# qwerty35/lsc_dr_planner

Hardware: AMD Instinct MI355X
Metric: qp_solves_per_sec (higher is better)
Workload: dtype f64; 1 GPU; configs[1]: 64 agents x M=5 x ~20 LSC half-spaces/seg, fp64 -- 64 agents/GPU x M=5 segments x 20 LSC neighbours (dim=3, forest swarm after 3 warm-up replans), fp64: dual active-set phase (one workgroup per QP) with the batched PDIP behind it for what it leaves; batch_seed=1000, precision=f64, row_format=f64, collective_backend=none (single process), agents_per_gpu=64, agents_total=64, ranks=1, distinct_devices=1, launch=single process, segments=5, lsc_neighbours=20, dim=3, rows_per_qp=1074, allgather=False, pipeline=False, hip_graph=False

## Files before the change

lsc_dr_planner_amd/csrc/lscqp_api.hip:

```cpp
#include <hip/hip_runtime.h>

#include <cmath>
#include <cstdio>
#include <cstdlib>
#include <cstring>
#include <algorithm>
#include <atomic>
#include <mutex>
#include <string>
#include <vector>

#include "lscqp_kernel.hpp"
#include "lscqp_launch.hpp"
#include "lscqp_staging.hpp"
#include "lscqp_internal.hpp"

#define LSCQP_DECL(M, D, E, S, W, X)                                                                                      \
    extern "C" hipError_t lscqp_launch_##M##_##D##_##E##_##S##_##W##_##X(const lscqp::DevClass*, int64_t, const lscqp_header*, \
                                                                  const lscqp_row*, const uint64_t*, const lscqp_box*,  \
                                                                  const double*, double*, double*, int32_t*, lscqp_info*, \
                                                                  hipStream_t);
LSCQP_INSTANCES(LSCQP_DECL)
#undef LSCQP_DECL

// ... 352 lines not shown
        c.dQ[i] = d->control_input_weight != 0
                      ? (double)(((long double)p_ref - (long double)d->control_input_weight * kQInt[i] * scl) /
                                 (long double)d->control_input_weight)
                      : 0.0;
    }
    for (int k = 0; k < 3; k++) {
        c.world_min[k] = d->world_min[k];
        c.world_max[k] = d->world_max[k];
    }
    c.tol = d->tol > 0 ? d->tol : 1e-10;
    c.max_iter = d->max_iter > 0 ? d->max_iter : 60;
    c.use_sfc = d->use_sfc;
    c.n_obs_max = 0;
    c.rows_f32 = d->row_format == LSCQP_ROWS_F32;
    c.repair = 0;
    c.rsfc = d->planner_mode == LSCQP_PLANNER_RSFC;
    if (d->active_set != LSCQP_ACTIVE_SET_DEFAULT && d->active_set != LSCQP_ACTIVE_SET_OFF && d->active_set != LSCQP_ACTIVE_SET_ONLY)
        return fail(LSCQP_ERR_INVALID_ARGUMENT, "active_set must be LSCQP_ACTIVE_SET_DEFAULT, _OFF or _ONLY");
    if (d->warm_start != LSCQP_WARM_DEFAULT && d->warm_start != LSCQP_WARM_TIGHT)
        return fail(LSCQP_ERR_INVALID_ARGUMENT, "warm_start must be LSCQP_WARM_DEFAULT or LSCQP_WARM_TIGHT");
    c.warm_mu0 = d->warm_start == LSCQP_WARM_TIGHT ? 1e-7 : LSCQP_WARM_MU0;
    c.warm_s0 = d->warm_start == LSCQP_WARM_TIGHT ? 0.003 : LSCQP_WARM_S0;
    c.warm_net = d->warm_start == LSCQP_WARM_TIGHT ? 0.6 : 0.0;
    return LSCQP_OK;
}

extern "C" const lscqp_class_desc* lscqp_class_desc_of_(lscqp_handle h) { return &h->desc; }
extern "C" uint64_t lscqp_handle_generation_(lscqp_handle h) { return h->generation; }

static bool das_upload(DasTables& D, int d) {
    if (D.dev[d]) {
        D.garbage.push_back({D.dev[d], d});
        D.dev[d] = nullptr;
    }
    if (D.host.empty()) return false;
    if (hipSetDevice(d) != hipSuccess) return false;
    double* p = nullptr;
    if (hipMalloc(&p, sizeof(double) * D.host.size()) != hipSuccess) return false;
    if (hipMemcpy(p, D.host.data(), sizeof(double) * D.host.size(), hipMemcpyHostToDevice) != hipSuccess) {
        (void)hipFree(p);
        return false;
    }
    D.dev[d] = p;
    D.dev_n[d] = D.host.size();
    D.dev_gen[d] = D.gen;
    return true;
}
static void das_refresh(lscqp_solver* s) {
    if (!s->das) return;
    std::lock_guard<std::mutex> lk(s->das->mu);
    DasTables& D = *s->das;
    const size_t nd = lscqp_das_build_tables(s->desc.M, s->es, s->desc.dt, s->desc.control_input_weight, s->desc.terminal_weight, nullptr);
    const size_t npair = lscqp_das_build_pairs(s->desc.M, s->desc.dim, s->desc.communication_range > 0, nullptr);
    std::vector<double> fresh(nd + 36 + npair, 0.0);
    if (s->desc.control_input_weight > 0 && s->desc.terminal_weight >= 0 &&
        lscqp_das_build_tables(s->desc.M, s->es, s->desc.dt, s->desc.control_input_weight, s->desc.terminal_weight, fresh.data()) == nd) {
        for (int i = 0; i < 36; i++) fresh[nd + i] = s->dev.dQ[i];
        static_assert(sizeof(double) == 2 * sizeof(int32_t), "two ints per table slot");
        lscqp_das_build_pairs(s->desc.M, s->desc.dim, s->desc.communication_range > 0, reinterpret_cast<int32_t*>(fresh.data() + nd + 36));
    } else {
        fresh.clear();
    }
    if (D.gen != 0 && fresh.size() == D.host.size() && (fresh.empty() || memcmp(fresh.data(), D.host.data(), sizeof(double) * fresh.size()) == 0))
        return;
    D.host.swap(fresh);
    D.gen++;
    int cur = 0;
    const bool have_cur = hipGetDevice(&cur) == hipSuccess;
    for (int d = 0; d < 64; d++)
        if (D.dev[d]) (void)das_upload(D, d);
    if (D.garbage.size() > DasTables::kMaxRetired) {
        for (const DasTables::Retired& g : D.garbage) {
            if (hipSetDevice(g.dev) == hipSuccess) {
                (void)hipDeviceSynchronize();
                (void)hipFree(g.p);
            }
        }
        D.garbage.clear();
    }
    if (have_cur) (void)hipSetDevice(cur);
}
static const double* das_device_table(lscqp_solver* s, hipStream_t stream, int* err = nullptr) {
    if (err) *err = 0;
    if (!s->das) return nullptr;
    int dev = 0;
    if (hipGetDevice(&dev) != hipSuccess || dev < 0 || dev >= 64) return nullptr;
    std::lock_guard<std::mutex> lk(s->das->mu);
    DasTables& D = *s->das;
    if (D.host.empty()) return nullptr;
    if (D.dev[dev] && D.dev_gen[dev] == D.gen) return D.dev[dev];
    hipStreamCaptureStatus cap = hipStreamCaptureStatusNone;
    const hipError_t qe = hipStreamIsCapturing(stream, &cap);
    if (qe != hipSuccess) (void)hipGetLastError();
    const bool capturing = qe != hipSuccess || cap != hipStreamCaptureStatusNone;
    if (capturing) {
        if (err) *err = 2;
        return nullptr;
    }
    if (!das_upload(D, dev)) {
        if (err) *err = 1;
        return nullptr;
    }
    return D.dev[dev];
}

static inline size_t row_bytes(lscqp_handle h) { return h->dev.rows_f32 ? sizeof(lscqp_row_f32) : sizeof(lscqp_row); }

extern "C" {

int lscqp_create(const lscqp_class_desc* desc, lscqp_handle* out) {
    if (!desc || !out) return fail(LSCQP_ERR_INVALID_ARGUMENT, "null argument");
    lscqp_solver* s = new lscqp_solver();
// ... 508 lines not shown
```

lsc_dr_planner_amd/csrc/lscqp_das.hip:

```cpp
#include <hip/hip_runtime.h>
#include <stdint.h>

#include <atomic>
#include <cmath>
#include <mutex>
#include <vector>

#include "lscqp_internal.hpp"
#include "lscqp_das.hpp"


extern "C" size_t lscqp_das_build_pairs(int M, int dim, int comm_on, int32_t* out) {
    const int P = 6 * M, NX = dim * P, NCP = M * (M - 1) / 2;
    const int oV = NX, oA = oV + dim * 5 * M, oC = oA + dim * 4 * M, NPAIR = lscqp_das::num_pairs(M, dim);
    if (!out) return (size_t)NPAIR;
    for (int r = 0; r < NPAIR; r++) {
        int type = 0, e0 = 0, e1 = 0, fam = 0, k = 0, m = 0, last = 0;
        if (r < oV) {
            k = r / P;
            const int cp = r - k * P;
            m = cp / 6, last = cp % 6 == 5;
            type = cp >= 3 ? 1 : 0, e0 = r, fam = 0;
        } else if (r < oA) {
            const int s = r - oV;
            k = s / (5 * M);
            const int rr = s - k * 5 * M, i = rr % 5;
            m = rr / 5;
            type = (m == 0 && i < 2) ? 0 : 2, e0 = k * P + 6 * m + i, fam = 1;
        } else if (r < oC) {
            const int s = r - oA;
            k = s / (4 * M);
            const int rr = s - k * 4 * M, i = rr % 4;
            m = rr / 4;
            type = (m == 0 && i < 1) ? 0 : 3, e0 = k * P + 6 * m + i, fam = 2;
        } else {
            const int s = r - oC;
            k = s / NCP;
            const int ci = s - k * NCP;
            int uu = 1;
            while (uu * (uu + 1) / 2 <= ci) uu++;
            const int up = ci - uu * (uu - 1) / 2;
            type = comm_on ? 4 : 0, e0 = k * P + 6 * (up + 1), e1 = k * P + 6 * uu + 5, fam = 3, m = 0;
        }
        out[2 * r] = (type << 24) | (e0 << 12) | e1;
        out[2 * r + 1] = fam | (k << 2) | (m << 4) | (last << 8) | ((fam == 0 && k == 2 && m == 0) ? 1 << 9 : 0);
    }
    return (size_t)NPAIR;
}

extern "C" size_t lscqp_das_build_tables(int M, int es, double dt, double w_c, double w_t, double* out) {
    const int P = 6 * M, NZA = 3 * (M - 1) + (es ? 1 : 3);
    const size_t stride = lscqp_das::table_stride(M);
    if (!out) return stride * (size_t)M;
    typedef long double ld;
    const ld q2s = 2.0L * (ld)w_c / ((ld)dt * dt * dt * dt * dt);
    static const int kq[6][6] = {{720, -1800, 1200, 0, 0, -120},  {-1800, 4800, -3600, 0, 600, 0}, {1200, -3600, 3600, -1200, 0, 0},
                                 {0, 0, -1200, 3600, -3600, 1200}, {0, 600, 0, -3600, 4800, -1800}, {-120, 0, 0, 1200, -1800, 720}};
    static const int tbm[3][3] = {{0, 0, 1}, {0, -1, 2}, {1, -4, 4}};
    std::vector<ld> Tm((size_t)P * NZA, 0.0L);
    for (int m = 0; m < M; m++) {
        const bool last = es && m == M - 1;
        for (int j = 0; j < 3; j++) Tm[(size_t)(6 * m + 3 + j) * NZA + 3 * m + (last ? 0 : j)] = 1.0L;
        if (m >= 1)
            for (int i = 0; i < 3; i++)
                for (int j = 0; j < 3; j++) Tm[(size_t)(6 * m + i) * NZA + 3 * (m - 1) + j] = (ld)tbm[i][j];
    }
    for (int ts = 1; ts <= M; ts++) {
        std::vector<ld> Hx((size_t)P * P, 0.0L);
        for (int m = 0; m < M; m++)
            for (int i = 0; i < 6; i++)
                for (int j = 0; j < 6; j++) Hx[(size_t)(6 * m + i) * P + 6 * m + j] += q2s * (ld)kq[i][j];
        for (int m = M - ts; m < M; m++) Hx[(size_t)(6 * m + 5) * P + 6 * m + 5] += 2.0L * (ld)w_t;
        std::vector<ld> HT((size_t)P * NZA, 0.0L), K0((size_t)NZA * NZA, 0.0L);
        for (int i = 0; i < P; i++)
            for (int l = 0; l < P; l++) {
                const ld h = Hx[(size_t)i * P + l];
                if (h == 0.0L) continue;
                for (int j = 0; j < NZA; j++) HT[(size_t)i * NZA + j] += h * Tm[(size_t)l * NZA + j];
            }
        for (int i = 0; i < P; i++)
            for (int a = 0; a < NZA; a++) {
                const ld t = Tm[(size_t)i * NZA + a];
                if (t == 0.0L) continue;
                for (int b = 0; b < NZA; b++) K0[(size_t)a * NZA + b] += t * HT[(size_t)i * NZA + b];
            }
        std::vector<ld> Lc((size_t)NZA * NZA, 0.0L);
        for (int j = 0; j < NZA; j++) {
            ld d = K0[(size_t)j * NZA + j];
            for (int l = 0; l < j; l++) d -= Lc[(size_t)j * NZA + l] * Lc[(size_t)j * NZA + l];
            if (!(d > 0.0L)) return 0;
            const ld dj = sqrtl(d);
            Lc[(size_t)j * NZA + j] = dj;
            for (int i = j + 1; i < NZA; i++) {
                ld s = K0[(size_t)i * NZA + j];
                for (int l = 0; l < j; l++) s -= Lc[(size_t)i * NZA + l] * Lc[(size_t)j * NZA + l];
                Lc[(size_t)i * NZA + j] = s / dj;
            }
        }
        std::vector<ld> X((size_t)NZA * P, 0.0L);
        for (int col = 0; col < P; col++) {
            for (int i = 0; i < NZA; i++) {
                ld s = Tm[(size_t)col * NZA + i];
// ... 98 lines not shown
```

lsc_dr_planner_amd/csrc/lscqp_das.hpp:

```cpp
#pragma once
#include <hip/hip_runtime.h>
#include <stdint.h>

#include "lscqp_kernel.hpp"
#include "lscqp_launch.hpp"

#pragma clang fp contract(on)

namespace lscqp_das {

using lscqp::DevClass;
using lscqp::KQ;

constexpr double kTolP = 1e-9;
constexpr double kTolD = 1e-9;
constexpr int kMaxK = 32;

__host__ __device__ constexpr size_t table_stride(int M) { return (size_t)(3 + 6 * M) * (size_t)(6 * M); }
__host__ __device__ constexpr int num_pairs(int M, int dim) { return dim * (6 * M + 5 * M + 4 * M + M * (M - 1) / 2); }

struct Layout {
    int P, NX, kmax, NPAIR;
    int o_hdr, o_sfc, o_c, o_cu, o_lam, o_plo, o_phi, o_pix, o_W, o_L, o_u, o_r, o_arhs, o_acoef, o_aint, o_red, o_ctl, o_wb, o_dq, o_C, o_rows, o_tl, n_stage, total;
    __host__ __device__ static constexpr Layout make(int M, int dim, int kmax, int cacheC, int stage_rows = 0) {
        Layout s{};
        s.P = 6 * M, s.NX = dim * s.P, s.kmax = kmax, s.NPAIR = num_pairs(M, dim);
        int o = 0;
        auto take = [&](int n) { const int at = o; o += (n + 1) & ~1; return at; };
        s.o_hdr = take(32);
        s.o_sfc = take(6 * M);
        s.o_c = take(3 * s.P), s.o_cu = take(s.NX), s.o_lam = take(s.NX);
        s.o_plo = take(s.NPAIR), s.o_phi = take(s.NPAIR), s.o_pix = take((s.NPAIR + 1) / 2);
        s.o_W = take((kmax + 1) * s.NX);
        s.o_L = take(kmax * (kmax + 1));
        s.o_u = take(kmax + 1), s.o_r = take(kmax + 4), s.o_arhs = take(kmax + 1);
        s.o_acoef = take(3 * (kmax + 1));
        s.o_aint = take(2 * (kmax + 1) + 2);
        s.o_red = take(2 * 24);
        s.o_ctl = take(8);
        s.o_wb = take(8);
        s.o_dq = take(36);
        s.o_C = take(cacheC ? s.P * s.P : 0);
        s.n_stage = stage_rows;
        s.o_rows = take(4 * stage_rows);
#ifdef LSCQP_DAS_TIMING
        s.o_tl = take(16);
#endif
        s.total = o;
        return s;
    }
};

__device__ __forceinline__ double wave_max(double v) { return lscqp::wave_max(v); }
__device__ __forceinline__ double wave_min(double v) { return -lscqp::wave_max(-v); }
__device__ __forceinline__ double wave_sum(double v) { return lscqp::wave_sum(v); }
template <int CTRL, int ROW_MASK>
__device__ __forceinline__ int dpp_min_i32(int v) {
    return min(v, __builtin_amdgcn_update_dpp(2147483647, v, CTRL, ROW_MASK, 0xf, false));
}
__device__ __forceinline__ int wave_min_i32(int v) {
    v = dpp_min_i32<0x111, 0xf>(v);
    v = dpp_min_i32<0x112, 0xf>(v);
    v = dpp_min_i32<0x114, 0xf>(v);
    v = dpp_min_i32<0x118, 0xf>(v);
    v = dpp_min_i32<0x142, 0xa>(v);
    v = dpp_min_i32<0x143, 0xc>(v);
    return __builtin_amdgcn_readlane(v, 63);
}
__device__ __forceinline__ void wave_argmin(double& v, int& id) {
    const double vm = wave_min(v);
    id = wave_min_i32((v == vm) ? id : 2147483647);
    v = vm;
// ... 154 lines not shown
```

lsc_dr_planner_amd/csrc/lscqp_das_body.inc:

```
#if LSCQP_DAS_PROLOGUE
#define DAS_CLS(f) ka_##f
#else
#define DAS_CLS(f) cls.f
#endif
    const int tid = threadIdx.x, lane = tid & 63, wv = tid >> 6;
#ifdef LSCQP_DAS_LAYOUT
    constexpr Layout L = LSCQP_DAS_LAYOUT;
#else
    const Layout L = Layout::make(M, dim, kmax, cacheC, stage_rows);
#endif
    DAS_T_DECL();
    const int P = L.P, NX = L.NX, NPAIR = L.NPAIR;
    const int kcap = L.kmax;
    double* const H_ = smem + L.o_hdr;
    double* const sfc_ = smem + L.o_sfc;
    double* const c_ = smem + L.o_c;
    double* const cu_ = smem + L.o_cu;
    double* const lam_ = smem + L.o_lam;
    double* const plo_ = smem + L.o_plo;
    double* const phi_ = smem + L.o_phi;
    int* const pix_ = reinterpret_cast<int*>(smem + L.o_pix);
    double* const W_ = smem + L.o_W;
    double* const Jm_ = smem + L.o_L;
    double* const u_ = smem + L.o_u;
    double* const r_ = smem + L.o_r;
    double* const arhs_ = smem + L.o_arhs;
    double* const acoef_ = smem + L.o_acoef;
    int* const aint_ = reinterpret_cast<int*>(smem + L.o_aint);
    double* const red_ = smem + L.o_red;
    double* const ctl_ = smem + L.o_ctl;
    double* const wb_ = smem + L.o_wb;
    double* const dq_ = smem + L.o_dq;
    double* const Cc_ = smem + L.o_C;
    double* const Sx_ = smem + L.o_rows;
    double* const Sy_ = Sx_ + L.n_stage;
    double* const Sz_ = Sy_ + L.n_stage;
    double* const Sb_ = Sz_ + L.n_stage;
    const int LDL = kcap + 1;
    int par = 0;

    if (!SCREEN && behind) {
        const int st_early = status_out[q];
        if ((behind & 1) && st_early == LSCQP_STATUS_OPTIMAL) LSCQP_DAS_END(kDasSolved);
        if ((behind & 2) && st_early == LSCQP_STATUS_INFEASIBLE) LSCQP_DAS_END(kDasInfeasible);
    }
#if LSCQP_DAS_PROLOGUE
    const lscqp_header* const hq = hdr + q;
    const bool use_sfc = ka_use_sfc != 0;
    constexpr int kNS = (72 + T - 1) / T;
    LSCQP_DAS_GLOBAL const double* const hsrc = (LSCQP_DAS_GLOBAL const double*)hq;
    LSCQP_DAS_GLOBAL const double* const ssrc = use_sfc ? ka_sfc + q * 6 * M : hsrc;
    double hw = hsrc[tid & 31];
    double sw[kNS];
#pragma unroll
    for (int i = 0; i < kNS; i++) sw[i] = ssrc[(use_sfc && tid + i * T < 6 * M) ? tid + i * T : 0];
    const double* const tab_end = tab + (size_t)M * table_stride(M);
    double dqw = tab_end[min(tid, 35)];
    constexpr int kPB = 4;
    const int2* const pairs_g = reinterpret_cast<const int2*>(tab_end + 36);
    int2 pwr[kPB];
#pragma unroll
    for (int u = 0; u < kPB; u++) pwr[u] = pairs_g[min(tid + u * T, NPAIR - 1)];
    const uint64_t roff_raw = *(ka_roffs ? ka_roffs + q : (LSCQP_DAS_GLOBAL const uint64_t*)hq);
    const int n_obs = hq->n_obs;
    __builtin_amdgcn_sched_barrier(0);
    const uint64_t roff = ka_roffs ? roff_raw : 0;
    const bool in_cap = !(n_obs > cap || n_obs < 0);
    const int nL = in_cap ? n_obs * P : 0;
    auto fetch_row = [&](int j, double& x, double& y, double& z, double& w) {
        if constexpr (F32) {
            const float4 f = reinterpret_cast<const float4*>(rows)[roff + (uint64_t)j];
            x = f.x, y = f.y, z = f.z, w = f.w;
        } else {
            const double4 d = *reinterpret_cast<const double4*>(&rows[roff + (uint64_t)j]);
            x = d.x, y = d.y, z = d.z, w = d.w;
        }
    };
    double px[kU], py[kU], pz[kU], pw[kU];
    {
        using RowT = std::conditional_t<F32, float4, double4>;
        const RowT* const rbase = nL > 0 ? reinterpret_cast<const RowT*>(rows) + roff : reinterpret_cast<const RowT*>(hq);
#pragma unroll
        for (int u = 0; u < kU; u++) {
            const int j = tid + u * T;
            const RowT d = rbase[j < nL ? j : 0];
            px[u] = nL > 0 ? (double)d.x : 0.0, py[u] = nL > 0 ? (double)d.y : 0.0, pz[u] = nL > 0 ? (double)d.z : 0.0, pw[u] = nL > 0 ? (double)d.w : -1.0;
        }
    }
    asm volatile("" : "+v"(hw), "+v"(dqw));
#pragma unroll
    for (int i = 0; i < kNS; i++) asm volatile("" : "+v"(sw[i]));
    if (tid < 32) H_[tid] = hw;
#pragma unroll
    for (int i = 0; i < kNS; i++)
        if (use_sfc && tid + i * T < 6 * M) sfc_[tid + i * T] = sw[i];
    if (tid < 36) dq_[tid] = dqw;
    if (tid == 0) {
        wb_[0] = ka_wb0, wb_[1] = ka_wb1, wb_[2] = ka_wb2, wb_[3] = ka_wb3, wb_[4] = ka_wb4, wb_[5] = ka_wb5;
        wb_[6] = ka_dt, wb_[7] = ka_q2s, ctl_[4] = ka_w_t, red_[44] = ka_w_c;
    }
    LSCQP_DAS_BARRIER();
#else
    const uint64_t roff = row_offsets ? row_offsets[q] : 0;
    constexpr int kPB = 4;
    const int2* const pairs_g = reinterpret_cast<const int2*>(tab + (size_t)M * table_stride(M) + 36);
    int2 pwr[kPB];
#pragma unroll
    for (int u = 0; u < kPB; u++) pwr[u] = pairs_g[min(tid + u * T, NPAIR - 1)];
    {
        const double* hsrc = reinterpret_cast<const double*>(hdr + q);
        const double* ssrc = reinterpret_cast<const double*>(sfc) + q * 6 * M;
        for (int e = tid; e < 32 + (cls.use_sfc ? 6 * M : 0); e += T) (e < 32 ? H_[e] : sfc_[e - 32]) = e < 32 ? hsrc[e] : ssrc[e - 32];
        if (tid >= 64 - 36 && tid < 64) dq_[tid - (64 - 36)] = tab[(size_t)M * table_stride(M) + (tid - (64 - 36))];
        if (tid < 6) {
            const double w = tid == 0 ? cls.world_min[0] : tid == 1 ? cls.world_min[1] : tid == 2 ? cls.world_min[2] : tid == 3 ? cls.world_max[0] : tid == 4 ? cls.world_max[1] : cls.world_max[2];
            wb_[tid] = w;
        }
    }
// ... 99 lines not shown
    for (int u = 0; u < kU; u++) px[u] = py[u] = pz[u] = 0.0, pw[u] = -1.0;
    if (nL > 0) {
#pragma unroll
        for (int u = 0; u < kU; u++) {
            const int j = tid + u * T;
            fetch_row(j < nL ? j : 0, px[u], py[u], pz[u], pw[u]);
        }
    }
#endif

    constexpr int kCPre = (NW == 4 && !PEEL && !SCREEN) ? 6 : 0;
    double cpre[kCPre > 0 ? kCPre : 1];
#if LSCQP_DAS_PROLOGUE
    const bool c_fits = kCPre > 0 && P * P <= kCPre * T;
    const bool c_prefetched = c_fits && cacheC;
#else
    const bool c_prefetched = kCPre > 0 && cacheC && P * P <= kCPre * T;
    const bool c_fits = c_prefetched;
#endif
    if constexpr (kCPre > 0) {
        if (c_fits) {
#pragma unroll
            for (int i = 0; i < kCPre; i++) {
                const int e = tid + i * T;
                cpre[i] = Cg[e < P * P ? e : 0];
            }
        }
    }
#if LSCQP_DAS_STEP_PATH & 2
#ifndef LSCQP_DAS_LAYOUT
#error "LSCQP_DAS_STEP_PATH & 2 needs the compile-time carve"
#endif
    static_assert(NW > 1, "the first pass's barrier publishes the table");
    constexpr bool kTableEarly = kCPre > 0 && L.P * L.P <= kCPre * T;
    static_assert(!kTableEarly || LSCQP_DAS_PROLOGUE, "the table is stored from cpre[]: it needs the prologue that always loads it");
#else
    constexpr bool kTableEarly = false;
#endif

    bool empty = false;
    const double hv_c = dt * 0.2, ha_c = dt * dt * 0.05;
#if LSCQP_DAS_STEP_PATH & 2048
#ifndef LSCQP_DAS_LAYOUT
#error "LSCQP_DAS_STEP_PATH & 2048 sizes its register copy from the compile-time carve"
#endif
    constexpr int kPR = (L.NPAIR + T - 1) / T;
    static_assert(kPR <= kPB && L.NPAIR <= kPB * T, "the section's first block of four slots holds every two-sided row of the shape");
    int tp_pk[kPR], tp_i0[kPR], tp_i1[kPR], tp_e0[kPR];
    double tp_a1[kPR], tp_a2[kPR], tp_lo[kPR], tp_hi[kPR];
#pragma unroll
    for (int u = 0; u < kPR; u++)
        tp_pk[u] = tp_i0[u] = tp_i1[u] = tp_e0[u] = 0, tp_a1[u] = tp_a2[u] = tp_lo[u] = tp_hi[u] = 0.0;
#endif
    for (int r0 = tid; r0 < NPAIR; r0 += kPB * T) {
        if (r0 != tid) {
#pragma unroll
            for (int u = 0; u < kPB; u++) pwr[u] = pairs_g[min(r0 + u * T, NPAIR - 1)];
        }
#pragma unroll
        for (int u = 0; u < kPB; u++) {
            if ((r0 - tid) + u * T >= NPAIR) break;
            const int r = r0 + u * T;
            const int w0 = pwr[u].x, w1 = pwr[u].y;
            const int fam = w1 & 3, k = (w1 >> 2) & 3, m = (w1 >> 4) & 15;
            const bool last = (w1 >> 8) & 1, rs = (w1 >> 9) & 1;
            const double ok_ = org[k], wlo = wb_[k], whi = wb_[3 + k], wpk = Hd->next_waypoint[k] - ok_;
            const double hv = Hd->vmax[k] * hv_c, ha = Hd->amax[k] * ha_c;
            double lo = wlo - ok_, hi = whi - ok_;
            if (DAS_CLS(rsfc) && rs) {
                lo = -100.0 - ok_;
                hi = 100.0 - ok_;
            }
            if (DAS_CLS(use_sfc)) {
                lo = fmax(lo, sfcl[m].bmin[k] - ok_);
                hi = fmin(hi, sfcl[m].bmax[k] - ok_);
            }
            const double clo = fmax(lo, fmax(-rho_pair, wpk - rho_wp)), chi = fmin(hi, fmin(rho_pair, wpk + rho_wp));
            lo = (comm_on && last) ? clo : lo;
            hi = (comm_on && last) ? chi : hi;
            const double hs = fam == 1 ? hv : fam == 2 ? ha : rho_pair;
            lo = fam == 0 ? lo : -hs;
            hi = fam == 0 ? hi : hs;
            if (r < NPAIR) {
                if (fam == 0 && (w0 >> 24) != 0 && lo > hi) empty = true;
                plo_[r] = lo, phi_[r] = hi;
                pix_[r] = w0;
            }
#if LSCQP_DAS_STEP_PATH & 2048
            if (u < kPR) {
                const int pk = r < NPAIR ? w0 : 0;
                const int type = pk >> 24, e0 = (pk >> 12) & 0xfff, e1 = pk & 0xfff;
                const int us = u < kPR ? u : 0;
                tp_pk[us] = pk;
                tp_i0[us] = (type == 4) ? e1 : e0 + max(type - 1, 0);
                tp_i1[us] = (type == 3) ? e0 + 1 : e0;
                tp_e0[us] = e0;
                tp_a1[us] = (type <= 1) ? 0.0 : (type == 3) ? -2.0 : -1.0;
                tp_a2[us] = (type == 3) ? 1.0 : 0.0;
                tp_lo[us] = lo, tp_hi[us] = hi;
            }
#endif
        }
    }
#pragma unroll
    for (int i = 0; i < NE; i++) {
        const int e = tid + i * T;
        if (e < NX) {
            const int k = fdiv(e, iP), cp = e - k * P;
            const double c1 = Hd->v0[k] * dt * 0.2;
            const double c2 = Hd->a0[k] * dt * dt * 0.05 + 2.0 * c1;
            const double fixv = (cp == 1) ? c1 : (cp == 2) ? c2 : 0.0;
            const double cv = fixv - c1 * tu1[i] - c2 * tu2[i] + wt2 * (Hd->goal[k] - org[k]) * tg1[i];
            c_[e] = cv;
            cu_[e] = cv;
        }
    }
    if (dim == 2)
        for (int e = tid; e < P; e += T) c_[2 * P + e] = 0.0;
#if LSCQP_DAS_STEP_PATH & 2
    {
        double2* const J2 = reinterpret_cast<double2*>(Jm_);
        for (int e = tid; e < kcap * LDL / 2; e += T) J2[e] = make_double2(0.0, 0.0);
    }
#endif
#if LSCQP_DAS_STEP_PATH & 8
    for (int e = tid; e < NX; e += T) lam_[e] = 0.0;
#endif
#if LSCQP_DAS_PROLOGUE
    const bool empty_w = __ballot(empty) != 0;
    if constexpr (NW > 1) {
        if (lane == 0) red_[20 + wv] = empty_w ? 1.0 : 0.0;
    }
    LSCQP_DAS_BARRIER();
    bool empty_g = empty_w;
    if constexpr (NW > 1) {
#if LSCQP_DAS_STEP_PATH & 64
        static_assert(NW == 4 && L.o_red % 2 == 0, "four ballots, two 16-byte words");
        const double2 b01 = *reinterpret_cast<const double2*>(red_ + 20), b23 = *reinterpret_cast<const double2*>(red_ + 22);
        empty_g = fmax(fmax(b01.x, b01.y), fmax(b23.x, b23.y)) != 0.0;
#else
        empty_g = false;
#pragma unroll
        for (int w = 0; w < NW; w++) empty_g = empty_g || red_[20 + w] != 0.0;
#endif
    }
#else
    if (tid == 0) ctl_[4] = 0.0;
    LSCQP_DAS_BARRIER();
    if (empty) ctl_[4] = 1.0;
    LSCQP_DAS_BARRIER();
#endif
#if LSCQP_DAS_PROLOGUE
    if (empty_g)
#else
    if (ctl_[4] != 0.0)
#endif
    {
        double ov = 0.0;
        if (wv == 0) {
            for (int r = lane; r < NPAIR; r += 64)
                if ((pix_[r] >> 24) != 0) ov = fmax(ov, plo_[r] - phi_[r]);
            ov = wave_max(ov);
        }
        infeasible_out(0, ov);
        LSCQP_DAS_END(kDasInfeasible);
    }
    DAS_T(1);

    auto translate = [&](int j, double x, double y, double z, double w, double& nx, double& ny, double& nz, double& b) -> bool {
        nx = x, ny = y, nz = (dim == 3) ? z : 0.0;
        b = (dim == 3) ? w - (x * org0 + y * org1 + z * org2) : w - (x * org0 + y * org1 + 0.0);
        return !(x * x + y * y + z * z < 1e-10) && (j - P * fdiv(j, iP)) >= 3;
    };
    auto load_row = [&](int j, double& nx, double& ny, double& nz, double& b) -> bool {
        if (rows_in_lds) {
            nx = Sx_[j], ny = Sy_[j], nz = Sz_[j], b = Sb_[j];
            return b != -1.0 || nx != 0.0 || ny != 0.0 || nz != 0.0;
        }
        double x, y, z, w;
// ... 972 lines not shown
```

lsc_dr_planner_amd/csrc/lscqp_fused.hip:

```cpp
#include <atomic>

#include "lscqp_kernel.hpp"
#include "lscqp_launch.hpp"
#define LSCQP_DAS_CYCLES das_fused_cycles
#include "lscqp_das.hpp"

#define LSCQP_FCAT_(a, b, c, d, e, f) a##b##_##c##_##d##_##e##_##f
#define LSCQP_FCAT(a, b, c, d, e, f) LSCQP_FCAT_(a, b, c, d, e, f)
#define LSCQP_FUSED_FN LSCQP_FCAT(lscqp_launch_fused_, LSCQP_M, LSCQP_DIM, LSCQP_ES, LSCQP_NSLOT, LSCQP_W)

namespace lscqp_das {

constexpr bool carve_fits(int M, int dim, int kmax, int stage_rows) {
    return sizeof(double) * (size_t)Layout::make(M, dim, kmax, 1, stage_rows).total <= lscqp::kMaxLdsBytes;
}
#if LSCQP_M == 10 && LSCQP_DIM == 3
#define LSCQP_FUSED_PROLOGUE 0
#else
#define LSCQP_FUSED_PROLOGUE 1
#endif
#ifndef LSCQP_FUSED_STEP_PATH
#if LSCQP_M == 5 || (LSCQP_M == 10 && LSCQP_DIM == 2)
#define LSCQP_FUSED_STEP_PATH (7 | 8 | 32 | 64 | 128 | 256 | 512 | 1024 | 2048 | 4096 | 8192)
#else
#define LSCQP_FUSED_STEP_PATH 0
#endif
#endif
template <int M, int DIM, bool ES, int NSLOT, int W>
struct FusedCarve {
    static constexpr int kStage = lscqp::Cfg<M, DIM, ES, NSLOT, W, (int)sizeof(double)>::MAX_OBS * 6 * M;
    static constexpr int KMAX = carve_fits(M, DIM, kMaxK, kStage) ? kMaxK : 20;
    static_assert(carve_fits(M, DIM, KMAX, kStage), "the fused phase's carve does not fit the CU's LDS");
};

template <int M, int DIM, bool ES, int NSLOT, int W>
__global__ __launch_bounds__(256, 1) void das_pdip_kernel(DevClass cls, int cap, int kmax, int max_steps, int cacheC, int stage_rows,
                                                          const double* __restrict__ tab, int64_t n, const lscqp_header* __restrict__ hdr,
                                                          const lscqp_row* __restrict__ rows, const uint64_t* __restrict__ row_offsets,
                                                          const lscqp_box* __restrict__ sfc, const double* __restrict__ x_init,
                                                          double* __restrict__ x_out, double* __restrict__ obj_out, int32_t* __restrict__ status_out,
                                                          lscqp_info* __restrict__ info_out) {
    static_assert(W >= 1 && W <= 4, "the interior-point instance runs on the first W of the workgroup's four wavefronts");
    extern __shared__ __attribute__((aligned(16))) double smem[];
#if LSCQP_FUSED_PROLOGUE
    LSCQP_DAS_KERNARGS();
    const int64_t k0 = blockIdx.x;
    if (k0 >= n) return;
    const int64_t q = ka_order ? (int64_t)ka_order[k0] : k0;
#else
    const int64_t k0 = blockIdx.x;
    if (k0 >= n) return;
    const int64_t q = cls.order ? (int64_t)cls.order[k0] : k0;
#endif
    int verdict = kDasSolved;
    {
        using FC = FusedCarve<M, DIM, ES, NSLOT, W>;
        constexpr int NW = 4, T = 64 * NW;
#ifdef LSCQP_FUSED_ROW_SLOTS
        constexpr int kU = LSCQP_FUSED_ROW_SLOTS;
#else
        constexpr int kU = (FC::kStage + T - 1) / T < 4 ? (FC::kStage + T - 1) / T : 4;
#endif
        constexpr bool F32 = false, SCREEN = false, PEEL = false;
        constexpr int dim = DIM, es = ES ? 1 : 0, behind = 0;
        constexpr int kMaxNL = FC::kStage;
        static_assert(kU == 4 || kMaxNL <= kU * T, "the row slots must cover the carve's staged rows");
        static_assert(kU >= 1, "an instance has rows");
#define LSCQP_DAS_END(verdict_)   \
    do {                          \
        verdict = (verdict_);     \
        goto phase_done;          \
    } while (0)
#define LSCQP_DAS_LAYOUT Layout::make(M, DIM, FC::KMAX, 1, FC::kStage)
#define LSCQP_DAS_PROLOGUE LSCQP_FUSED_PROLOGUE
#define LSCQP_DAS_STEP_PATH LSCQP_FUSED_STEP_PATH
// ... 56 lines not shown
```

lsc_dr_planner_amd/csrc/lscqp_internal.hpp:

```cpp
#ifndef LSCQP_INTERNAL_HPP
#define LSCQP_INTERNAL_HPP

#include <hip/hip_runtime.h>
#include <stddef.h>
#include <stdint.h>

#include "../../include/lscqp.h"

namespace lscqp {
struct DevClass;
}
namespace {
struct SolvePlan;
}

extern "C" {

int lscqp_set_error_(int code, const char* msg);
int lscqp_need_device_(void);
int lscqp_launch_result_(hipError_t e);
const lscqp_class_desc* lscqp_class_desc_of_(lscqp_handle h);
uint64_t lscqp_handle_generation_(lscqp_handle h);
int lscqp_has_other_order_(lscqp_handle h, int64_t n, int32_t n_obs_max);
int lscqp_debug_reload_knobs_(lscqp_handle h);
int lscqp_debug_set_knob_(lscqp_handle h, const char* name, int value);
int lscqp_check_missions_(int64_t n_total, int32_t n_missions, const int64_t* mission_offsets);
int lscqp_solve_batch_device_internal_(lscqp_handle h, int64_t n, int32_t n_obs_max, const lscqp_header* d_hdr, const lscqp_row* d_rows,
                                       const uint64_t* d_row_offsets, const lscqp_box* d_sfc, const double* d_x_init, double* d_x_out, double* d_obj_out,
                                       int32_t* d_status_out, lscqp_info* d_info_out, int32_t retry, int32_t part, const int32_t* d_order, void* stream,
                                       int* deferred);
int lscqp_debug_solve_plan_(lscqp_handle h, int64_t n, int32_t n_obs_max, int32_t retry, int32_t part, int32_t has_x_init, int32_t has_order,
                            int32_t deferred, int32_t n_cu, int32_t tables_available, SolvePlan* out);
int lscqp_debug_prescreen_twin_(lscqp_handle h, int64_t n, int32_t n_obs_max, const lscqp_header* hdr, const lscqp_row* rows, const uint64_t* row_offsets,
                                const lscqp_box* sfc, lscqp_prescreen_cert* cert_out);

int lscqp_work_table_(int M, int D, int E, int S, int W, int X, double* out24);

int lscqp_generic_supports(int M, int dim, int es);
int lscqp_generic_max_obstacles(int M, int dim, int es);
size_t lscqp_generic_lds_bytes(int M, int dim, int es, int n_obs_max);
hipError_t lscqp_launch_generic(const lscqp::DevClass* cls, int M, int dim, int es, int64_t n, const lscqp_header* hdr, const lscqp_row* rows,
                                const uint64_t* row_offsets, const lscqp_box* sfc, const double* x_init, double* x_out, double* obj_out,
                                int32_t* status_out, lscqp_info* info_out, hipStream_t stream);

size_t lscqp_das_build_tables(int M, int es, double dt, double w_c, double w_t, double* out);
size_t lscqp_das_build_pairs(int M, int dim, int comm_on, int32_t* out);
size_t lscqp_das_lds_bytes(int M, int dim, int kmax, int cacheC, int stage_rows);
int lscqp_das_blocks_per_cu(int M, int dim, int kmax, int rows_f32);
hipError_t lscqp_launch_das(const lscqp::DevClass* cls, int M, int dim, int es, int cap, int threads, int kmax, int max_steps, int cacheC,
                            int stage_rows, int screen, const double* d_tab, int64_t n, const lscqp_header* hdr, const lscqp_row* rows, const uint64_t* row_offsets,
                            const lscqp_box* sfc, const double* x_init, double* x_out, double* obj_out, int32_t* status_out,
                            lscqp_info* info_out, hipStream_t stream);

hipError_t lscqp_launch_prescreen(const lscqp::DevClass* cls, int M, int dim, int cap, int64_t n, const lscqp_header* hdr, const lscqp_row* rows,
                                  const uint64_t* row_offsets, const lscqp_box* sfc, const double* x_init, lscqp_prescreen_cert* cert_out,
                                  double* x_out, double* obj_out, int32_t* status_out, lscqp_info* info_out, hipStream_t stream);
int lscqp_prescreen_host_twin_(const lscqp::DevClass* cls, int M, int dim, int cap, int64_t n, const lscqp_header* hdr, const void* rows,
                               const uint64_t* row_offsets, const lscqp_box* sfc, lscqp_prescreen_cert* cert_out);

int lscqp_generate_lsc_raw_(int mode, int M, int dim, int64_t n_agents, int32_t n_obs, int64_t first_agent,
                            const double* d_traj, const double* d_own_traj, const int32_t* d_neighbours, const double* d_radius,
                            const double* d_downwash, const double* d_goal, const double* d_goal_all, int rows_f32,
                            int32_t n_obs_total, int32_t slot0, lscqp_row* d_rows_out, void* stream);
int lscqp_generate_clsc_obstacles_raw_(int M, int dim, double dt, double obs_downwash_threshold, int64_t n_agents, int32_t n_dyn,
                                       int64_t first_agent, const double* d_traj, const int32_t* d_obstacle_ids,
                                       const lscqp_obstacle* d_obstacles, const double* d_obstacle_goal, const double* d_radius,
                                       const double* d_goal, int rows_f32, int32_t n_obs_total, int32_t slot0, lscqp_row* d_rows_out,
                                       void* stream);
int lscqp_generate_constraints_own_(lscqp_handle h, int32_t mode, int64_t n_agents, int32_t n_obs, int64_t first_agent,
                                    const double* d_traj, const double* d_own_traj, const int32_t* d_neighbours, const double* d_radius,
                                    const double* d_downwash, const double* d_goal_all, lscqp_row* d_rows_out, int32_t n_obs_total,
                                    int32_t slot0, void* stream);

int lscqp_optimize_goal_fin_device_(lscqp_handle h, int64_t n, lscqp_header* d_hdr, const lscqp_row* d_rows, const uint64_t* d_row_offsets,
                                    const lscqp_box* d_sfc, int32_t* d_status_out, double fin_dt, void* stream);

int lscqp_commit_validate_raw_(int M, int dim, int use_sfc, double dt, int64_t n, double time_step, double z_2d, const int32_t* d_qp_status,
                               const double* d_x_new, const double* d_x_init, double* d_x_plan, double* d_goal, const lscqp_header* d_hdr,
                               const lscqp_box* d_sfc, int32_t* d_valid, double* d_state, void* stream);

int lscqp_map_device_(lscqp_map mp);
uint64_t lscqp_map_generation_(lscqp_map mp);
int lscqp_map_raw_(lscqp_map mp, double* res, float* world_min, float* world_max, int* key0, int* dims, const int32_t** d_nearest, int* device);
hipError_t lscsfc_launch_throughput_(const void* view, int mode, int M, int64_t n, const double* d_points, const double* d_radius,
                                     lscqp_box* d_sfc, int32_t* d_status_out, void* stream);
hipError_t lscsfc_launch_throughput_worlds_(const void* view, int mode, int M, int64_t n, const double* d_points, const double* d_radius,
                                            lscqp_box* d_sfc, int32_t* d_status_out, const void* d_table, const int32_t* d_world_of, void* stream);
int lscsfc_throughput_max_cells_(void);
int lscqp_worlds_count_(lscqp_worlds w);
lscqp_map lscqp_worlds_map_(lscqp_worlds w, int k);
uint64_t lscqp_worlds_generation_(lscqp_worlds w);
int lscqp_worlds_refresh_(lscqp_worlds w);
const char* lscqp_worlds_shape_difference_(lscqp_worlds w, lscqp_map mp);

int lscqp_grid_reserve_missions_(lscqp_grid g, int64_t n, int32_t n_missions);

int lscqp_record_create_(lscqp_handle h, int64_t n_total, int32_t n_missions, const int64_t* mission_offsets,
                         const int64_t* d_offsets_borrowed, int32_t n_samples, double record_time_step, double time_step, double z_2d,
                         const lscqp_record_desc* desc, lscqp_record* out);
// ... 11 lines not shown
```

Before: 7.852 million QP/s.

## Precompute per-pair constraint fields on host and hoist workspace zero-fills

Builds a per-pair field plane on the host (indices, coefficients, LDS byte offsets, family flags) and stores it after the packed pair words in the device table. In the M=5 fused DAS kernel, each thread loads its records once into registers and fills the two-sided bounds without decoding bits or running a strided loop. The zero-fills of the factor, lam and the unused c third for dim 2 move ahead of the first barrier in the prologue. The cost is more global loads per thread (four 16-byte words per pair), more table memory and more registers, which may reduce occupancy.

```diff
diff --git a/lsc_dr_planner_amd/csrc/lscqp_api.hip b/lsc_dr_planner_amd/csrc/lscqp_api.hip
--- a/lsc_dr_planner_amd/csrc/lscqp_api.hip
+++ b/lsc_dr_planner_amd/csrc/lscqp_api.hip
@@ -428,12 +428,14 @@
     DasTables& D = *s->das;
     const size_t nd = lscqp_das_build_tables(s->desc.M, s->es, s->desc.dt, s->desc.control_input_weight, s->desc.terminal_weight, nullptr);
     const size_t npair = lscqp_das_build_pairs(s->desc.M, s->desc.dim, s->desc.communication_range > 0, nullptr);
-    std::vector<double> fresh(nd + 36 + npair, 0.0);
+    const size_t o_fields = lscqp_das_pair_fields_offset(s->desc.M, s->desc.dim);
+    std::vector<double> fresh(o_fields + npair * (size_t)LSCQP_DAS_PAIR_FIELDS_DOUBLES, 0.0);
     if (s->desc.control_input_weight > 0 && s->desc.terminal_weight >= 0 &&
         lscqp_das_build_tables(s->desc.M, s->es, s->desc.dt, s->desc.control_input_weight, s->desc.terminal_weight, fresh.data()) == nd) {
         for (int i = 0; i < 36; i++) fresh[nd + i] = s->dev.dQ[i];
         static_assert(sizeof(double) == 2 * sizeof(int32_t), "two ints per table slot");
         lscqp_das_build_pairs(s->desc.M, s->desc.dim, s->desc.communication_range > 0, reinterpret_cast<int32_t*>(fresh.data() + nd + 36));
+        lscqp_das_build_pair_fields(s->desc.M, s->desc.dim, s->desc.communication_range > 0, fresh.data() + o_fields);
     } else {
         fresh.clear();
     }
diff --git a/lsc_dr_planner_amd/csrc/lscqp_das.hip b/lsc_dr_planner_amd/csrc/lscqp_das.hip
--- a/lsc_dr_planner_amd/csrc/lscqp_das.hip
+++ b/lsc_dr_planner_amd/csrc/lscqp_das.hip
@@ -3,6 +3,7 @@
 
 #include <atomic>
 #include <cmath>
+#include <cstring>
 #include <mutex>
 #include <vector>
 
@@ -48,6 +49,31 @@
     return (size_t)NPAIR;
 }
 
+static_assert(4 * sizeof(lscqp_das::PairWord0) == LSCQP_DAS_PAIR_FIELDS_DOUBLES * sizeof(double), "what the class's block is sized for");
+extern "C" size_t lscqp_das_pair_fields_offset(int M, int dim) { return lscqp_das::pair_fields_offset(M, dim); }
+extern "C" size_t lscqp_das_build_pair_fields(int M, int dim, int comm_on, void* out) {
+    const size_t n = lscqp_das_build_pairs(M, dim, comm_on, nullptr);
+    if (!out) return n;
+    std::vector<int32_t> w(2 * n);
+    lscqp_das_build_pairs(M, dim, comm_on, w.data());
+    char* const plane = static_cast<char*>(out);
+    memset(plane, 0, 64 * n);
+    for (size_t r = 0; r < n; r++) {
+        const int w0 = w[2 * r], w1 = w[2 * r + 1];
+        const int fam = w1 & 3, k = (w1 >> 2) & 3, m = (w1 >> 4) & 15;
+        const int type = w0 >> 24, e0 = (w0 >> 12) & 0xfff, e1 = w0 & 0xfff;
+        lscqp_das::PairWord0 g0 = {w0, (type == 4) ? e1 : e0 + (type - 1 > 0 ? type - 1 : 0), (type == 3) ? e0 + 1 : e0, e0};
+        lscqp_das::PairWord1 g1 = {(type <= 1) ? 0.0 : (type == 3) ? -2.0 : -1.0, (type == 3) ? 1.0 : 0.0};
+        lscqp_das::PairWord2 g2 = {8 * k, 8 * (6 * m + k), fam, (w1 >> 8) & 1};
+        lscqp_das::PairWord3 g3 = {(w1 >> 9) & 1, (fam == 0 && type != 0) ? 1 : 0, {0, 0}};
+        memcpy(plane + 16 * (0 * n + r), &g0, 16);
+        memcpy(plane + 16 * (1 * n + r), &g1, 16);
+        memcpy(plane + 16 * (2 * n + r), &g2, 16);
+        memcpy(plane + 16 * (3 * n + r), &g3, 16);
+    }
+    return n;
+}
+
 extern "C" size_t lscqp_das_build_tables(int M, int es, double dt, double w_c, double w_t, double* out) {
     const int P = 6 * M, NZA = 3 * (M - 1) + (es ? 1 : 3);
     const size_t stride = lscqp_das::table_stride(M);
diff --git a/lsc_dr_planner_amd/csrc/lscqp_das.hpp b/lsc_dr_planner_amd/csrc/lscqp_das.hpp
--- a/lsc_dr_planner_amd/csrc/lscqp_das.hpp
+++ b/lsc_dr_planner_amd/csrc/lscqp_das.hpp
@@ -18,6 +18,29 @@
 
 __host__ __device__ constexpr size_t table_stride(int M) { return (size_t)(3 + 6 * M) * (size_t)(6 * M); }
 __host__ __device__ constexpr int num_pairs(int M, int dim) { return dim * (6 * M + 5 * M + 4 * M + M * (M - 1) / 2); }
+
+__host__ __device__ constexpr size_t pair_fields_offset(int M, int dim) {
+    return (size_t)M * table_stride(M) + 36 + (size_t)((num_pairs(M, dim) + 1) & ~1);
+}
+struct PairWord0 {
+    int32_t pk;
+    int32_t i0, i1, e0;
+};
+struct PairWord1 {
+    double a1, a2;
+};
+struct PairWord2 {
+    int32_t ko;
+    int32_t so;
+    int32_t fam;
+    int32_t last;
+};
+struct PairWord3 {
+    int32_t rs;
+    int32_t ivl;
+    int32_t pad[2];
+};
+static_assert(sizeof(PairWord0) == 16 && sizeof(PairWord1) == 16 && sizeof(PairWord2) == 16 && sizeof(PairWord3) == 16, "16-byte words");
 
 struct Layout {
     int P, NX, kmax, NPAIR;
diff --git a/lsc_dr_planner_amd/csrc/lscqp_das_body.inc b/lsc_dr_planner_amd/csrc/lscqp_das_body.inc
--- a/lsc_dr_planner_amd/csrc/lscqp_das_body.inc
+++ b/lsc_dr_planner_amd/csrc/lscqp_das_body.inc
@@ -59,11 +59,54 @@
     constexpr int kPB = 4;
     const int2* const pairs_g = reinterpret_cast<const int2*>(tab_end + 36);
     int2 pwr[kPB];
+#if !(LSCQP_DAS_STEP_PATH & 16384)
 #pragma unroll
     for (int u = 0; u < kPB; u++) pwr[u] = pairs_g[min(tid + u * T, NPAIR - 1)];
+#endif
     const uint64_t roff_raw = *(ka_roffs ? ka_roffs + q : (LSCQP_DAS_GLOBAL const uint64_t*)hq);
     const int n_obs = hq->n_obs;
     __builtin_amdgcn_sched_barrier(0);
+#if LSCQP_DAS_STEP_PATH & 16384
+#ifndef LSCQP_DAS_LAYOUT
+#error "LSCQP_DAS_STEP_PATH & 16384 sizes the thread's records from the compile-time carve"
+#endif
+    static_assert((LSCQP_DAS_STEP_PATH & 2048) != 0, "the records feed the two-sided rows' registers");
+    constexpr int kPF = (L.NPAIR + T - 1) / T;
+    static_assert(kPF <= kPB && sizeof(PairWord0) == sizeof(int4), "one block of slots; 16-byte words");
+    const int4* const pfields_g = reinterpret_cast<const int4*>(tab + pair_fields_offset(M, dim));
+    int4 pfa[kPF], pfc[kPF];
+    double2 pfb[kPF];
+    int2 pfd[kPF];
+#pragma unroll
+    for (int u = 0; u < kPF; u++) {
+        const int4* const w = pfields_g + min(tid + u * T, NPAIR - 1);
+        pfa[u] = w[0], pfb[u] = *reinterpret_cast<const double2*>(w + NPAIR), pfc[u] = w[2 * NPAIR], pfd[u] = *reinterpret_cast<const int2*>(w + 3 * NPAIR);
+    }
+#endif
+#if LSCQP_DAS_STEP_PATH & 65536
+#ifndef LSCQP_DAS_LAYOUT
+#error "LSCQP_DAS_STEP_PATH & 65536 takes its trip counts from the compile-time carve"
+#endif
+    static_assert((LSCQP_DAS_STEP_PATH & 2) != 0 && (LSCQP_DAS_STEP_PATH & 8) != 0 && LSCQP_DAS_PROLOGUE != 0 && NW > 1,"the fills of bits 2 and 8, moved; the first barrier publishes them");
+    static_assert(L.o_hdr + 32 <= L.o_sfc && L.o_sfc + 6 * (L.P / 6) <= L.o_c && L.o_c + 3 * L.P <= L.o_cu && L.o_cu + L.NX <= L.o_lam && L.o_lam + L.NX <= L.o_plo,
+                  "H_, sfc_ in front of c_; lam_ behind c_ and cu_, in front of the two-sided rows");
+    static_assert(L.o_W + (L.kmax + 1) * L.NX <= L.o_L && L.o_L + L.kmax * (L.kmax + 1) <= L.o_u && L.o_u < L.o_red && L.o_red + 48 <= L.o_ctl &&
+                      L.o_ctl + 8 <= L.o_wb && L.o_wb + 8 <= L.o_dq && L.o_L % 2 == 0 && (L.kmax * (L.kmax + 1)) % 2 == 0,
+                  "the factor behind W_, in front of red_, ctl_, wb_ and dq_; 16-byte stores");
+    {
+        constexpr int nJ2 = L.kmax * (L.kmax + 1) / 2;
+        double2* const J2 = reinterpret_cast<double2*>(Jm_);
+#pragma unroll
+        for (int i = 0; i < (nJ2 + T - 1) / T; i++) J2[min(tid + i * T, nJ2 - 1)] = make_double2(0.0, 0.0);
+#pragma unroll
+        for (int i = 0; i < (L.NX + T - 1) / T; i++) lam_[min(tid + i * T, L.NX - 1)] = 0.0;
+        if constexpr (L.NX == 2 * L.P) {
+#pragma unroll
+            for (int i = 0; i < (L.P + T - 1) / T; i++) c_[2 * L.P + min(tid + i * T, L.P - 1)] = 0.0;
+        }
+    }
+    __builtin_amdgcn_sched_barrier(0);
+#endif
     const uint64_t roff = ka_roffs ? roff_raw : 0;
     const bool in_cap = !(n_obs > cap || n_obs < 0);
     const int nL = in_cap ? n_obs * P : 0;
@@ -269,6 +312,43 @@
     for (int u = 0; u < kPR; u++)
         tp_pk[u] = tp_i0[u] = tp_i1[u] = tp_e0[u] = 0, tp_a1[u] = tp_a2[u] = tp_lo[u] = tp_hi[u] = 0.0;
 #endif
+#if LSCQP_DAS_STEP_PATH & 16384
+    static_assert(kPF == kPR, "a record per register slot");
+    auto lds_at = [](const double* base, int bytes) { return *reinterpret_cast<const double*>(reinterpret_cast<const char*>(base) + bytes); };
+#pragma unroll
+    for (int u = 0; u < kPR; u++) {
+        const int r = tid + u * T;
+        const bool has = r < NPAIR;
+        const int fam = pfc[u].z;
+        const bool last = pfc[u].w != 0, rs = pfd[u].x != 0;
+        const int ko = pfc[u].x, so = pfc[u].y;
+        const double ok_ = lds_at(org, ko), wlo = lds_at(wb_, ko), whi = lds_at(wb_ + 3, ko), wpk = lds_at(Hd->next_waypoint, ko) - ok_;
+        const double hv = lds_at(Hd->vmax, ko) * hv_c, ha = lds_at(Hd->amax, ko) * ha_c;
+        double lo = wlo - ok_, hi = whi - ok_;
+        if (DAS_CLS(rsfc) && rs) {
+            lo = -100.0 - ok_;
+            hi = 100.0 - ok_;
+        }
+        if (DAS_CLS(use_sfc)) {
+            lo = fmax(lo, lds_at(sfc_, so) - ok_);
+            hi = fmin(hi, lds_at(sfc_ + 3, so) - ok_);
+        }
+        const double clo = fmax(lo, fmax(-rho_pair, wpk - rho_wp)), chi = fmin(hi, fmin(rho_pair, wpk + rho_wp));
+        lo = (comm_on && last) ? clo : lo;
+        hi = (comm_on && last) ? chi : hi;
+        const double hs = fam == 1 ? hv : fam == 2 ? ha : rho_pair;
+        lo = fam == 0 ? lo : -hs;
+        hi = fam == 0 ? hi : hs;
+        if (has) {
+            if (pfd[u].y != 0 && lo > hi) empty = true;
+            plo_[r] = lo, phi_[r] = hi;
+            pix_[r] = pfa[u].x;
+        }
+        tp_pk[u] = has ? pfa[u].x : 0, tp_i0[u] = has ? pfa[u].y : 0, tp_i1[u] = has ? pfa[u].z : 0, tp_e0[u] = has ? pfa[u].w : 0;
+        tp_a1[u] = has ? pfb[u].x : 0.0, tp_a2[u] = has ? pfb[u].y : 0.0;
+        tp_lo[u] = lo, tp_hi[u] = hi;
+    }
+#else
     for (int r0 = tid; r0 < NPAIR; r0 += kPB * T) {
         if (r0 != tid) {
 #pragma unroll
@@ -319,6 +399,7 @@
 #endif
         }
     }
+#endif
 #pragma unroll
     for (int i = 0; i < NE; i++) {
         const int e = tid + i * T;
@@ -332,16 +413,20 @@
             cu_[e] = cv;
         }
     }
+#if !(LSCQP_DAS_STEP_PATH & 65536)
     if (dim == 2)
         for (int e = tid; e < P; e += T) c_[2 * P + e] = 0.0;
-#if LSCQP_DAS_STEP_PATH & 2
+#endif
+#if (LSCQP_DAS_STEP_PATH & 2) && !(LSCQP_DAS_STEP_PATH & 65536)
     {
         double2* const J2 = reinterpret_cast<double2*>(Jm_);
         for (int e = tid; e < kcap * LDL / 2; e += T) J2[e] = make_double2(0.0, 0.0);
     }
 #endif
 #if LSCQP_DAS_STEP_PATH & 8
+#if !(LSCQP_DAS_STEP_PATH & 65536)
     for (int e = tid; e < NX; e += T) lam_[e] = 0.0;
+#endif
 #endif
 #if LSCQP_DAS_PROLOGUE
     const bool empty_w = __ballot(empty) != 0;
diff --git a/lsc_dr_planner_amd/csrc/lscqp_fused.hip b/lsc_dr_planner_amd/csrc/lscqp_fused.hip
--- a/lsc_dr_planner_amd/csrc/lscqp_fused.hip
+++ b/lsc_dr_planner_amd/csrc/lscqp_fused.hip
@@ -20,7 +20,9 @@
 #define LSCQP_FUSED_PROLOGUE 1
 #endif
 #ifndef LSCQP_FUSED_STEP_PATH
-#if LSCQP_M == 5 || (LSCQP_M == 10 && LSCQP_DIM == 2)
+#if LSCQP_M == 5
+#define LSCQP_FUSED_STEP_PATH (7 | 8 | 32 | 64 | 128 | 256 | 512 | 1024 | 2048 | 4096 | 8192 | 16384 | 65536)
+#elif LSCQP_M == 10 && LSCQP_DIM == 2
 #define LSCQP_FUSED_STEP_PATH (7 | 8 | 32 | 64 | 128 | 256 | 512 | 1024 | 2048 | 4096 | 8192)
 #else
 #define LSCQP_FUSED_STEP_PATH 0
diff --git a/lsc_dr_planner_amd/csrc/lscqp_internal.hpp b/lsc_dr_planner_amd/csrc/lscqp_internal.hpp
--- a/lsc_dr_planner_amd/csrc/lscqp_internal.hpp
+++ b/lsc_dr_planner_amd/csrc/lscqp_internal.hpp
@@ -45,6 +45,9 @@
 
 size_t lscqp_das_build_tables(int M, int es, double dt, double w_c, double w_t, double* out);
 size_t lscqp_das_build_pairs(int M, int dim, int comm_on, int32_t* out);
+#define LSCQP_DAS_PAIR_FIELDS_DOUBLES 8
+size_t lscqp_das_build_pair_fields(int M, int dim, int comm_on, void* out);
+size_t lscqp_das_pair_fields_offset(int M, int dim);
 size_t lscqp_das_lds_bytes(int M, int dim, int kmax, int cacheC, int stage_rows);
 int lscqp_das_blocks_per_cu(int M, int dim, int kmax, int rows_f32);
 hipError_t lscqp_launch_das(const lscqp::DevClass* cls, int M, int dim, int es, int cap, int threads, int kmax, int max_steps, int cacheC,
```

New measurement: 7.887 million QP/s (median of 6 runs). No clear change (+0.5%).
